# ttwang0303/Adaptive-RGBD-Localization-Mappig

Hardware: AMD Instinct MI355X
Metric: frames/sec (extract+match+RANSAC-PnP) @640x480, 2000 kp (higher is better)
Workload: dtype u8/i32 (extract, match), f32+f64 (ransac, pnp)

## Files before the change

adaptive-rgbd-localization-mappig_amd/csrc/k_extract.hip:

```cpp
#include "odo_device.h"
#include "odo_internal.h"
#ifdef FS_STATS
#include <cstdio>
#endif

#ifndef ODO_EXTRACT_PRIO
#define ODO_EXTRACT_PRIO 0
#endif
#define EXTRACT_PRIO() \
    if (ODO_EXTRACT_PRIO) __builtin_amdgcn_s_setprio(ODO_EXTRACT_PRIO)

namespace odo {

__global__ void __launch_bounds__(256) k_gray(const uint8_t* __restrict__ bgr, uint8_t* __restrict__ pyr,
                                              int w, int h, int pitch, size_t in_stride, size_t pyr_stride) {
    EXTRACT_PRIO();
    const int f = blockIdx.y;
    const int q = blockIdx.x * blockDim.x + threadIdx.x;
    const uint8_t* src = bgr + (size_t)f * in_stride;
    uint8_t* dst = pyr + (size_t)f * pyr_stride;
    const int npix = w * h;
    const int p0 = q * 4;
    if (p0 >= npix) return;
    const int y = p0 / w, x = p0 - y * w;
// ... 35 lines not shown
    const int nrow = min(rb, dh - y0);
    const int t = threadIdx.x;
    uint8_t* base = pyr + (size_t)f * pyr_stride;
    const int sy_lo = yt[y0].sy0, sy_hi = yt[y0 + nrow - 1].sy1;
    const int srows = sy_hi - sy_lo + 1;
    const int nq = (dw + 3) >> 2;
    ResizeX* xs = reinterpret_cast<ResizeX*>(rz_lds);
    uint8_t* rows = rz_lds + (size_t)nq * 4 * sizeof(ResizeX);
    for (int i = t; i < dw; i += 256) xs[i] = xt[i];
    {
        const uint4* src = reinterpret_cast<const uint4*>(base + src_off + (size_t)sy_lo * spitch);
        uint4* dstl = reinterpret_cast<uint4*>(rows);
        const int n16 = srows * (spitch >> 4);
        for (int i = t; i < n16; i += 256) dstl[i] = src[i];
    }
    __syncthreads();
    const float inv_nq = 1.0f / (float)nq;
    const int items = nrow * nq;
    for (int it = t; it < items; it += 256) {
        const int r = (int)(((float)it + 0.5f) * inv_nq);
        const int q = it - r * nq;
        const ResizeY Y = yt[y0 + r];
        const uint8_t* r0 = rows + (uint32_t)__umul24((uint32_t)(Y.sy0 - sy_lo), (uint32_t)spitch);
        const uint8_t* r1 = rows + (uint32_t)__umul24((uint32_t)(Y.sy1 - sy_lo), (uint32_t)spitch);
        const uint32_t b0 = (uint32_t)Y.b0, b1 = (uint32_t)Y.b1;
        uint32_t packed = 0;
#pragma unroll
        for (int j = 0; j < 4; j++) {
            const int dx = 4 * q + j;
            if (dx < dw) {
                const ResizeX X = xs[dx];
                const uint32_t a0 = (uint32_t)X.a0, a1 = (uint32_t)X.a1;
                const uint32_t h0 = __umul24(r0[X.sx0], a0) + __umul24(r0[X.sx1], a1);
                const uint32_t h1 = __umul24(r1[X.sx0], a0) + __umul24(r1[X.sx1], a1);
                const uint32_t v = (__umul24(h0, b0) + __umul24(h1, b1) + (1u << 21)) >> 22;
                packed |= min(v, 255u) << (8 * j);
            }
        }
        *reinterpret_cast<uint32_t*>(base + dst_off + (size_t)(y0 + r) * dpitch + 4 * q) = packed;
    }
}

constexpr int kCircleDx[16] = {0, 1, 2, 3, 3, 3, 2, 1, 0, -1, -2, -3, -3, -3, -2, -1};
constexpr int kCircleDy[16] = {3, 3, 2, 1, 0, -1, -2, -3, -3, -3, -2, -1, 0, 1, 2, 3};
#define FS_TH 256
#define FS_RING 512
#define FS_RSTRIDE (FS_RING + 8)
#define FS_CL 1024

ODO_INLINE void wave_lds_sync() {
    __builtin_amdgcn_fence(__ATOMIC_RELEASE, "wavefront");
    __builtin_amdgcn_wave_barrier();
    __builtin_amdgcn_fence(__ATOMIC_ACQUIRE, "wavefront");
}

#ifdef FS_STATS
__device__ unsigned long long fs_stats[8];
#define FS_STAT(i, v) atomicAdd(&fs_stats[i], (unsigned long long)(v))
#else
#define FS_STAT(i, v) ((void)0)
#endif
ODO_INLINE uint32_t fs_msb_mask(uint32_t b4) {
    return ((b4 & 1u) << 7) | ((b4 & 2u) << 14) | ((b4 & 4u) << 21) | ((b4 & 8u) << 28);
}
ODO_INLINE int wave_incl_scan(int x) {
    x += __builtin_amdgcn_update_dpp(0, x, 0x111, 0xf, 0xf, true);
    x += __builtin_amdgcn_update_dpp(0, x, 0x112, 0xf, 0xf, true);
    x += __builtin_amdgcn_update_dpp(0, x, 0x114, 0xf, 0xf, true);
    x += __builtin_amdgcn_update_dpp(0, x, 0x118, 0xf, 0xf, true);
    x += __builtin_amdgcn_update_dpp(0, x, 0x142, 0xa, 0xf, false);
    x += __builtin_amdgcn_update_dpp(0, x, 0x143, 0xc, 0xf, false);
    return x;
}
struct FastMisc {
    int ncl, ovf, nl;
    int tot[FS_NCM], retry[FS_NCM];
};

__global__ void __launch_bounds__(FS_TH) k_fast_seg(const uint8_t* __restrict__ pyr, size_t pyr_stride,
                                                   const FastSeg* __restrict__ segs, const LevelDesc* __restrict__ lv,
                                                   uint32_t* __restrict__ cand, int* __restrict__ cand_cnt, int ncells,
                                                   int cell_cap, int ini_th, int min_th, FastLds LO) {
    EXTRACT_PRIO();
    extern __shared__ __attribute__((aligned(16))) uint8_t fs_lds[];
    const FastSeg G = segs[blockIdx.x];
    const int f = blockIdx.y;
    const int t = threadIdx.x, lane = t & 63, wave = t >> 6;
    uint8_t* const roi = fs_lds;
    const uint32_t* const roi32 = reinterpret_cast<const uint32_t*>(fs_lds);
    uint8_t* const score = fs_lds + LO.img;
    uint16_t* const ring = reinterpret_cast<uint16_t*>(fs_lds + LO.ring) + wave * FS_RSTRIDE;
    uint16_t* const clist = reinterpret_cast<uint16_t*>(fs_lds + LO.clist);
    uint32_t* const bits = reinterpret_cast<uint32_t*>(fs_lds + LO.bits);
    int* const cnt = reinterpret_cast<int*>(fs_lds + LO.cnt);
    uint2* const qlist = reinterpret_cast<uint2*>(fs_lds + LO.qlist);
    FastMisc& M = *reinterpret_cast<FastMisc*>(fs_lds + LO.misc);
    const LevelDesc L = lv[G.level];
    const int R = G.rows, cols = G.cols, BW = G.bw, wcell = G.wcell, nc = G.ncell;
    constexpr int RS = FS_RS, RS4 = RS >> 2;
    const int sh = G.x0 & 15;
    {
        const uint4* src = reinterpret_cast<const uint4*>(pyr + (size_t)f * pyr_stride + L.off +
                                                          (size_t)G.y0 * L.pitch + (G.x0 & ~15));
        const int nw = (sh + cols + 15) >> 4, p16 = L.pitch >> 4;
        const int rstep = FS_TH / nw, k = t % nw, r0 = t / nw;
        if (r0 < rstep)
            for (int r = r0; r < R; r += rstep)
                reinterpret_cast<uint4*>(roi + r * RS)[k] = src[__umul24((uint32_t)r, (uint32_t)p16) + (uint32_t)k];
        for (int i = t; i < (R * RS) >> 4; i += FS_TH) reinterpret_cast<uint4*>(score)[i] = uint4{0, 0, 0, 0};
        for (int i = t; i < R * BW; i += FS_TH) bits[i] = 0;
        for (int i = t; i < R * FS_NCM; i += FS_TH) cnt[i] = 0;
        if (t == 0) M.ncl = 0, M.ovf = 0;
    }
    const int drows = R - 6;
    const int m0 = (sh + 3) >> 2, m1 = (sh + cols - 4) >> 2;
    {
        const uint32_t mlo = (0xFu << (sh + 3 - 4 * m0)) & 0xFu, mhi = (1u << (sh + cols - 3 - 4 * m1)) - 1u;
        if (t <= m1 - m0) {
            const int m = m0 + t;
            qlist[t] = uint2{fs_msb_mask((t == 0 ? mlo : 0xFu) & (m == m1 ? mhi : 0xFu)), 4u * (uint32_t)m};
        }
    }
    __syncthreads();
    const float inv_w = 1.0f / (float)wcell;
    uint32_t* const out = cand + ((size_t)f * ncells + G.ci0) * cell_cap;
    typedef short s16x2 __attribute__((ext_vector_type(2)));
    for (int pass = 0; pass < 2; pass++) {
        const int th = pass == 0 ? ini_th : min_th;
        const int thc = th < 0 ? 0 : (th > 255 ? 255 : th);
        const int NL = pass == 0 ? m1 - m0 + 1 : M.nl;
        const int items = drows > 0 && cols > 6 && NL > 0 ? drows * NL : 0;
        if (t == 0) FS_STAT(pass, items);
        {
            const s16x2 thv = {(short)thc, (short)thc};
            const float inl = NL > 0 ? 1.0f / (float)NL : 0.0f, inl_h = 0.5f * inl;
            int head = 0, tail = 0;
            auto seg_test = [&](int h, int n) {
                const int i0 = 2 * lane, i1 = i0 + 1;
                bool c0 = false, c1 = false;
                int o0 = 0, o1 = 0;
                if (i0 < n) {
                    o0 = ring[(h + i0) & (FS_RING - 1)];
                    o1 = i1 < n ? ring[(h + i1) & (FS_RING - 1)] : o0;
                    const s16x2 vv = {(short)roi[o0], (short)roi[o1]};
                    int a0 = o0 - 3 * RS - 3, a1 = o1 - 3 * RS - 3;
                    asm("" : "+v"(a0), "+v"(a1));
                    const uint8_t* const q0 = roi + a0;
                    const uint8_t* const q1 = roi + a1;
                    s16x2 d[16];
#pragma unroll
                    for (int k = 0; k < 16; k++) {
                        const int off = (kCircleDy[k] + 3) * RS + kCircleDx[k] + 3;
                        s16x2 c;
                        c.x = (short)q0[off];
                        c.y = (short)q1[off];
                        d[k] = vv - c;
                    }
                    s16x2 mn2[8], mx2[8], mn4[8], mx4[8];
#pragma unroll
                    for (int q = 0; q < 8; q++) {
                        const int j = 2 * q + 1;
                        mn2[q] = __builtin_elementwise_min(d[j], d[(j + 1) & 15]);
                        mx2[q] = __builtin_elementwise_max(d[j], d[(j + 1) & 15]);
                    }
#pragma unroll
                    for (int q = 0; q < 8; q++) {
                        mn4[q] = __builtin_elementwise_min(mn2[q], mn2[(q + 1) & 7]);
                        mx4[q] = __builtin_elementwise_max(mx2[q], mx2[(q + 1) & 7]);
                    }
                    s16x2 dk = s16x2{-32768, -32768}, br = s16x2{32767, 32767};
#pragma unroll
                    for (int q = 0; q < 8; q++) {
                        const int k = 2 * q;
                        const s16x2 m8 = __builtin_elementwise_min(mn4[q], mn4[(q + 2) & 7]);
                        const s16x2 x8 = __builtin_elementwise_max(mx4[q], mx4[(q + 2) & 7]);
                        dk = __builtin_elementwise_max(
                            dk, __builtin_elementwise_min(m8, __builtin_elementwise_max(d[k], d[(k + 9) & 15])));
                        br = __builtin_elementwise_min(
                            br, __builtin_elementwise_max(x8, __builtin_elementwise_min(d[k], d[(k + 9) & 15])));
                    }
                    const s16x2 sc = __builtin_elementwise_max(dk, -br);
                    c0 = sc.x > thc;
                    c1 = i1 < n && sc.y > thc;
                    if (c0) score[o0] = (uint8_t)(sc.x - 1);
                    if (c1) score[o1] = (uint8_t)(sc.y - 1);
                }
                const uint64_t b0 = __ballot(c0), b1 = __ballot(c1);
                const int nco = __popcll(b0) + __popcll(b1);
                if (lane == 0) FS_STAT(3, 1);
                if (nco) {
                    int cb = 0;
                    if (lane == 0) cb = atomicAdd(&M.ncl, nco);
                    cb = __shfl(cb, 0);
                    const int pre = (int)__builtin_amdgcn_mbcnt_hi((uint32_t)(b0 >> 32), __builtin_amdgcn_mbcnt_lo((uint32_t)b0, 0)) +
                                    (int)__builtin_amdgcn_mbcnt_hi((uint32_t)(b1 >> 32), __builtin_amdgcn_mbcnt_lo((uint32_t)b1, 0));
                    const int p0 = cb + pre, p1 = p0 + (c0 ? 1 : 0);
                    if (c0) { if (p0 < FS_CL) clist[p0] = (uint16_t)o0; else M.ovf = 1; }
                    if (c1) { if (p1 < FS_CL) clist[p1] = (uint16_t)o1; else M.ovf = 1; }
                }
            };
            for (int base = wave * 64; base < items; base += FS_TH) {
                uint32_t pass4 = 0;
                int qoff = 0;
                const int it = base + lane;
                if (it < items) {
                    const int ii = (int)__builtin_fmaf((float)it, inl, inl_h);
                    const int kk = it - __mul24(ii, NL);
                    const uint2 e = qlist[kk];
                    int wb = (int)__umul24((uint32_t)ii, (uint32_t)RS) + (int)e.y;
                    asm("" : "+v"(wb));
                    qoff = wb + 3 * RS;
                    const uint32_t* w = reinterpret_cast<const uint32_t*>(roi + wb);
                    const uint32_t Cw = w[3 * RS4], Uw = w[0], Dw = w[6 * RS4];
                    const uint32_t Lw = __builtin_amdgcn_alignbyte(Cw, w[3 * RS4 - 1], 1);
                    const uint32_t Rw = __builtin_amdgcn_alignbyte(w[3 * RS4 + 1], Cw, 3);
                    uint32_t hm[2];
#pragma unroll
                    for (int hh = 0; hh < 2; hh++) {
                        const uint32_t sel = hh ? 0x0c030c02u : 0x0c010c00u;
                        s16x2 v, a0, a4, a8, a12;
                        *reinterpret_cast<uint32_t*>(&v) = __builtin_amdgcn_perm(0u, Cw, sel);
                        *reinterpret_cast<uint32_t*>(&a0) = __builtin_amdgcn_perm(0u, Dw, sel);
                        *reinterpret_cast<uint32_t*>(&a4) = __builtin_amdgcn_perm(0u, Rw, sel);
                        *reinterpret_cast<uint32_t*>(&a8) = __builtin_amdgcn_perm(0u, Uw, sel);
                        *reinterpret_cast<uint32_t*>(&a12) = __builtin_amdgcn_perm(0u, Lw, sel);
                        const s16x2 dk = __builtin_elementwise_max(__builtin_elementwise_min(a0, a8),
                                                                   __builtin_elementwise_min(a4, a12));
                        const s16x2 bk = __builtin_elementwise_min(__builtin_elementwise_max(a0, a8),
                                                                   __builtin_elementwise_max(a4, a12));
                        const s16x2 t1 = dk - (v - thv), t2 = (v + thv) - bk;
                        hm[hh] = *reinterpret_cast<const uint32_t*>(&t1) | *reinterpret_cast<const uint32_t*>(&t2);
                    }
                    pass4 = __builtin_amdgcn_perm(hm[1], hm[0], 0x07050301u) & e.x;
                }
                uint32_t pos = (uint32_t)tail;
#pragma unroll
                for (int k = 0; k < 4; k++) {
                    const bool sv = (pass4 >> (8 * k + 7)) & 1u;
                    const uint64_t bk = __ballot(sv);
                    const uint32_t slot =
                        __builtin_amdgcn_mbcnt_hi((uint32_t)(bk >> 32), __builtin_amdgcn_mbcnt_lo((uint32_t)bk, pos)) &
                        (FS_RING - 1);
                    uint32_t at;
                    asm("v_cndmask_b32_e64 %0, %1, %2, %3" : "=v"(at) : "v"((uint32_t)FS_RING), "v"(slot), "s"(bk));
                    ring[at] = (uint16_t)(qoff + k);
                    pos += (uint32_t)__popcll(bk);
                }
                tail = (int)pos;
                if (tail - head >= 128) {
                    wave_lds_sync();
                    do {
                        seg_test(head, 128);
                        head += 128;
                    } while (tail - head >= 128);
                    wave_lds_sync();
                }
            }
            if (lane == 0) FS_STAT(2, tail);
            if (tail > head) {
                wave_lds_sync();
                seg_test(head, tail - head);
            }
        }
        __syncthreads();
        const bool ovf = M.ovf != 0;
        const int ncl = min(M.ncl, FS_CL);
        if (t == 0) FS_STAT(4, M.ncl), FS_STAT(5, ovf ? 1 : 0);
        auto locate = [&](int o, int& r, int& xs, int& jl, int& xl, int& xh) {
            r = o / RS;
            xs = (o - r * RS) - sh;
            jl = (int)(((float)(xs - 3) + 0.5f) * inv_w);
            xl = 3 + jl * wcell;
            xh = min(xl + wcell, cols - 3);
        };
        auto nms = [&](int o) {
            int so = o - RS - 1;
            asm("" : "+v"(so));
            const uint8_t* const sb = score + so;
            const int sc = sb[RS + 1];
            int r, xs, jl, xl, xh;
            locate(o, r, xs, jl, xl, xh);
            const int nmid = max((int)sb[1], (int)sb[2 * RS + 1]);
            const int nl = max(max((int)sb[0], (int)sb[RS]), (int)sb[2 * RS]);
            const int nr = max(max((int)sb[2], (int)sb[RS + 2]), (int)sb[2 * RS + 2]);
            const int nb = max(nmid, max(xs - 1 >= xl ? nl : 0, xs + 1 < xh ? nr : 0));
            if (sc > nb) {
                atomicOr(&bits[r * BW + (xs >> 5)], 1u << (xs & 31));
                atomicAdd(&cnt[r * FS_NCM + jl], 1);
            }
        };
        auto scan = [&](auto&& fn) {
            for (int it = t; it < items; it += FS_TH) {
                const int ii2 = it / NL, kk2 = it - ii2 * NL;
                const uint2 e = qlist[kk2];
                const uint32_t msk = e.x;
                const int qo = (3 + ii2) * RS + (int)e.y;
                for (int b = 0; b < 4; b++)
                    if (((msk >> (8 * b + 7)) & 1u) && score[qo + b]) fn(qo + b);
            }
        };
        if (!ovf)
            for (int i = t; i < ncl; i += FS_TH) nms(clist[i]);
        else
            scan(nms);
        __syncthreads();
        for (int j = wave; j < nc; j += FS_TH / 64) {
            if (pass == 1 && !M.retry[j]) continue;
            const int r = 3 + lane;
            const int v = lane < drows ? cnt[r * FS_NCM + j] : 0;
            int incl = v;
#pragma unroll
            for (int o = 1; o < 64; o <<= 1) {
                const int y = __shfl_up(incl, o);
                if (lane >= o) incl += y;
            }
            if (lane < drows) cnt[r * FS_NCM + j] = incl - v;
            if (lane == 63) M.tot[j] = incl;
        }
        __syncthreads();
        auto place = [&](int o) {
            int r, xs, jl, xl, xh;
            locate(o, r, xs, jl, xl, xh);
            const uint32_t* row = bits + r * BW;
            if (!((row[xs >> 5] >> (xs & 31)) & 1u)) return;
            int rank = cnt[r * FS_NCM + jl];
            const int wl = xl >> 5, nwd = (xs >> 5) - wl;
            const uint32_t hm = (1u << (xs & 31)) - 1u;
#pragma unroll
            for (int i = 0; i < 4; i++) {
                uint32_t v = row[wl + i];
                if (i == 0) v &= ~0u << (xl & 31);
                v &= i < nwd ? ~0u : (i == nwd ? hm : 0u);
                rank += __builtin_popcount(v);
            }
            if (rank < cell_cap)
                out[(size_t)jl * cell_cap + rank] = ((uint32_t)score[o] << 24) |
                                                    ((uint32_t)(r + G.y0 - 16) << 12) | (uint32_t)(xs + G.x0 - 16);
        };
        if (!ovf)
            for (int i = t; i < ncl; i += FS_TH) place(clist[i]);
        else
            scan(place);
        if (pass == 0) {
            if (t < nc) M.retry[t] = M.tot[t] == 0;
            __syncthreads();
            if (t < nc && M.retry[t]) FS_STAT(6, 1);
            if (t == 0) FS_STAT(7, nc);
            if (t < nc) {
                const int xa = sh + 3 + t * wcell, xe = sh + min(3 + (t + 1) * wcell, cols - 3);
                if (M.retry[t]) {
                    int at = 0;
                    for (int j = 0; j < t; j++)
                        if (M.retry[j]) {
                            const int ja = sh + 3 + j * wcell, je = sh + min(3 + (j + 1) * wcell, cols - 3);
                            at += ((je - 1) >> 2) - (ja >> 2) + 1;
                        }
                    for (int m = xa >> 2; m <= (xe - 1) >> 2; m++) {
                        const int lo = max(xa - 4 * m, 0), hi = min(xe - 4 * m, 4);
                        qlist[at++] = uint2{fs_msb_mask((0xFu << lo) & ((1u << hi) - 1u)), 4u * (uint32_t)m};
                    }
                } else {
                    cand_cnt[(size_t)f * ncells + G.ci0 + t] = min(M.tot[t], cell_cap);
                }
            }
            if (t == 0) {
                int n = 0;
                for (int j = 0; j < nc; j++)
                    if (M.retry[j]) {
                        const int ja = sh + 3 + j * wcell, je = sh + min(3 + (j + 1) * wcell, cols - 3);
                        n += ((je - 1) >> 2) - (ja >> 2) + 1;
                    }
                M.nl = n;
                M.ncl = 0;
                M.ovf = 0;
            }
            __syncthreads();
            if (M.nl == 0) return;
        } else if (t < nc && M.retry[t]) {
            cand_cnt[(size_t)f * ncells + G.ci0 + t] = min(M.tot[t], cell_cap);
        }
    }
}

struct ONode {
    int16_t x0, y0, x1, y1;
    int32_t cnt;
    int32_t seq;
};

#ifndef OT_THREADS
#define OT_THREADS 256
#endif

#ifndef OT_KB
#define OT_KB 8
#endif
#ifndef OT_RANK_MAX
#define OT_RANK_MAX 512
#endif
#ifdef ODO_OCTREE_PROFILE
#define OT_NSTAMP 48
__device__ unsigned long long g_ot_stamp[2][OT_NSTAMP];
#define OT_STAMP(tag)                                                                                   \
    do {                                                                                                \
        if (threadIdx.x == 0 && s_vars[8] >= 0 && s_vars[8] < OT_NSTAMP)                                \
            g_ot_stamp[s_vars[9]][s_vars[8]++] = ((unsigned long long)(tag) << 56) | (wall_clock64() & 0xFFFFFFFFFFFFFFull); \
    } while (0)
#else
#define OT_STAMP(tag) ((void)0)
#endif
#ifndef OT_HIST_WAVE0
#define OT_HIST_WAVE0 1
#endif
enum { OT_LDK = 1, OT_LDN = 2 };
template <bool RES, int LD, typename F>
ODO_INLINE void ot_pass(int n, int t, uint32_t (&rk)[OT_KB], int (&rn)[OT_KB], const uint32_t* keys, int32_t* knode,
                        F&& f) {
    if constexpr (RES) {
#pragma unroll
        for (int u = 0; u < OT_KB; u++)
            if (t + u * OT_THREADS < n) f(t + u * OT_THREADS, rk[u], rn[u]);
    } else {
        for (int k0 = t; k0 < n; k0 += OT_THREADS * OT_KB) {
#pragma unroll
            for (int u = 0; u < OT_KB; u++) {
                const int k = k0 + u * OT_THREADS;
                rn[u] = -1;
                if (k < n) {
                    if (LD & OT_LDK) rk[u] = keys[k];
                    if (LD & OT_LDN) rn[u] = knode[k];
                }
            }
#pragma unroll
            for (int u = 0; u < OT_KB; u++) {
                const int k = k0 + u * OT_THREADS;
                if (k < n) {
                    int node = rn[u];
                    f(k, rk[u], node);
                    if (node != rn[u]) knode[k] = node;
                }
            }
        }
    }
}

ODO_INLINE int block_exclusive_scan(int v, int* tmp, int* total);

ODO_INLINE int ot_gather(const uint32_t* __restrict__ cand, const int* __restrict__ cand_cnt, size_t cell0, int nc,
                         int cell_cap, uint32_t* dst, int cap, int* scan) {
    const int t = threadIdx.x;
    int n = 0;
    for (int cb = 0; cb < nc; cb += OT_THREADS) {
        const int c = cb + t;
        const int cnt = c < nc ? cand_cnt[cell0 + c] : 0;
        int tot;
        const int ex = block_exclusive_scan(cnt, scan, &tot);
        if (c < nc) {
// ... 1441 lines not shown
```

adaptive-rgbd-localization-mappig_amd/csrc/k_finalize.hip:

```cpp
#include "odo_device.h"
#include "odo_internal.h"
#ifndef ODO_EXTRACT_PRIO
#define ODO_EXTRACT_PRIO 0
#endif
#include "../../include/odo_orb_pattern.h"

namespace odo {

typedef float f32x2 __attribute__((ext_vector_type(2)));

__constant__ float4 c_patf[256];
__constant__ uint32_t c_pat8[256];
__constant__ int c_umax16[16];

#define RND_MAGIC 12582912.0f
#define RND_BITS 0x4B400000u

#define FIN_KPW 4

#define FL_IC_W 9
#define FL_IC_N (31 * FL_IC_W)
#define FL_BR_W 10
#define FL_BR_N (37 * FL_BR_W)
#define FL_KP_RAW FL_BR_N
#define FL_KP_DW (((FL_KP_RAW + 15) / 32) * 32 + 16)
template <int NW>
__global__ void __launch_bounds__(64 * NW) k_finalize_lds(const uint8_t* __restrict__ pyr, const uint8_t* __restrict__ blur,
                                                      size_t pyr_stride, const LevelDesc* __restrict__ lv, int nlevels,
                                                      const uint32_t* __restrict__ okp, const int* __restrict__ ocnt,
                                                      int okp_stride, orb_kp* __restrict__ kps, uint8_t* __restrict__ desc,
                                                      int* __restrict__ nkp, int kp_cap) {
    if (ODO_EXTRACT_PRIO) __builtin_amdgcn_s_setprio(ODO_EXTRACT_PRIO);
    __shared__ uint64_t s_bal[NW][16];
    __shared__ __attribute__((aligned(16))) uint32_t s_disc[16][12];
    __shared__ __attribute__((aligned(16))) uint32_t s_patch[NW * FIN_KPW][FL_KP_DW];
    for (int d = threadIdx.x; d < 128; d += 64 * NW) {
        const int av = d >> 3, i = d & 7;
        const int um = c_umax16[av];
        uint32_t m = 0;
#pragma unroll
        for (int bb = 0; bb < 4; bb++) {
            const int u = 4 * i + bb - 15;
            if (u >= -um && u <= um) m |= 0xffu << (8 * bb);
        }
        s_disc[av][i] = m;
    }
    int bx = blockIdx.x, f = blockIdx.y;
    {
        const int total = gridDim.x * gridDim.y;
        if ((total & 7) == 0) {
            const int h = blockIdx.x + blockIdx.y * gridDim.x;
            const int lid = (h & 7) * (total >> 3) + (h >> 3);
            bx = lid % gridDim.x;
            f = lid / gridDim.x;
        }
    }
    const int wave = threadIdx.x >> 6, lane = threadIdx.x & 63;
    const int g = lane >> 4, sub = lane & 15;
    const int kslot = wave * FIN_KPW + g;
    const int idx = bx * (NW * FIN_KPW) + kslot;
    int lvl = -1, k = 0, acc = 0;
    for (int i = 0; i < nlevels; i++) {
        const int c = ocnt[f * nlevels + i];
        if (lvl < 0 && idx < acc + c) {
            lvl = i;
            k = idx - acc;
        }
        acc += c;
    }
    const int total = acc < kp_cap ? acc : kp_cap;
    if (bx == 0 && threadIdx.x == 0) nkp[f] = total;
    if (bx * (NW * FIN_KPW) >= total) return;
    const bool valid = lvl >= 0 && idx < kp_cap;
    const LevelDesc L = lv[valid ? lvl : 0];
    const uint32_t key = valid ? okp[((size_t)f * nlevels + lvl) * okp_stride + k] : (16u | (16u << 12));
    const int kx = (int)(key & 0xfff) + 16, ky = (int)((key >> 12) & 0xfff) + 16;
    const float resp = (float)(key >> 24);
    constexpr int IC_STEPS = 7, BR_STEPS = 13;
    uint2 vbr[BR_STEPS];
    uint32_t* P = s_patch[kslot];
    const int sh = (kx - 15) & 3, sh2 = (kx - 18) & 3;
    const bool glane = sub < 15;
    const int ir = sub / 3, ic = sub - 3 * ir;
    const int br = sub / 5, bc = sub - 5 * br;
    {
        const uint8_t* fpyr = pyr + (size_t)f * pyr_stride;
        const uint8_t* fblur = blur + (size_t)f * pyr_stride;
        const uint32_t pitch = (uint32_t)L.pitch;
        uint3 v[IC_STEPS];
        {
            const uint32_t o0 = (uint32_t)L.off + (uint32_t)(ky - 15) * pitch + (uint32_t)(kx - 15 - sh);
            uint32_t o = o0 + (uint32_t)ir * pitch + 12u * (uint32_t)ic;
#pragma unroll
            for (int j = 0; j < IC_STEPS; j++) {
                const bool ok = j + 1 < IC_STEPS || ir == 0;
                v[j] = *reinterpret_cast<const uint3*>(fpyr + (ok ? o : o0));
                o += 5u * pitch;
            }
        }
        {
            const uint32_t o0 = (uint32_t)L.off + (uint32_t)(ky - 18) * pitch + (uint32_t)(kx - 18 - sh2);
            uint32_t o = o0 + (uint32_t)br * pitch + 8u * (uint32_t)bc;
#pragma unroll
            for (int j = 0; j < BR_STEPS; j++) {
                const bool ok = j + 1 < BR_STEPS || br == 0;
                vbr[j] = *reinterpret_cast<const uint2*>(fblur + (ok ? o : o0));
                o += 3u * pitch;
            }
        }
        {
            uint32_t* d = P + ir * FL_IC_W + 3 * ic;
#pragma unroll
            for (int j = 0; j < IC_STEPS; j++) {
                if (glane && (j + 1 < IC_STEPS || ir == 0)) {
                    d[0] = v[j].x;
                    d[1] = v[j].y;
                    d[2] = v[j].z;
                }
                d += 5 * FL_IC_W;
            }
        }
    }
    __syncthreads();
    int m10, m01;
    {
        const bool has1 = sub < 15;
        const int v0 = sub - 15, v1 = has1 ? sub + 1 : 0;
        const uint32_t* r0 = P + (v0 + 15) * FL_IC_W;
        const uint32_t* r1 = P + (v1 + 15) * FL_IC_W;
        uint32_t w0[9], w1[9];
#pragma unroll
        for (int i = 0; i < 9; i++) {
            w0[i] = r0[i];
            w1[i] = r1[i];
        }
        const uint4* M0 = reinterpret_cast<const uint4*>(s_disc[-v0]);
        const uint4* M1 = reinterpret_cast<const uint4*>(s_disc[v1]);
        const uint4 a0 = M0[0], a1 = M0[1], b0 = M1[0], b1 = M1[1];
        const uint32_t z = has1 ? 0xffffffffu : 0u;
        const uint32_t mk0[8] = {a0.x, a0.y, a0.z, a0.w, a1.x, a1.y, a1.z, a1.w};
        const uint32_t mk1[8] = {b0.x & z, b0.y & z, b0.z & z, b0.w & z, b1.x & z, b1.y & z, b1.z & z, b1.w & z};
        uint32_t s0 = 0, s1 = 0, t = 0;
#pragma unroll
        for (int i = 0; i < 8; i++) {
            const uint32_t U = (uint32_t)(4 * i + 1) | ((uint32_t)(4 * i + 2) << 8) | ((uint32_t)(4 * i + 3) << 16) |
                               ((uint32_t)(4 * i + 4) << 24);
            const uint32_t d0 = __builtin_amdgcn_alignbyte(w0[i + 1], w0[i], sh) & mk0[i];
            const uint32_t d1 = __builtin_amdgcn_alignbyte(w1[i + 1], w1[i], sh) & mk1[i];
            s0 = __builtin_amdgcn_udot4(d0, 0x01010101u, s0, false);
            s1 = __builtin_amdgcn_udot4(d1, 0x01010101u, s1, false);
            t = __builtin_amdgcn_udot4(d0, U, t, false);
            t = __builtin_amdgcn_udot4(d1, U, t, false);
        }
        m10 = (int)t - 16 * (int)(s0 + s1);
        m01 = v0 * (int)s0 + v1 * (int)s1;
    }
#pragma unroll
    for (int off = 8; off > 0; off >>= 1) {
        m10 += __shfl_xor(m10, off);
        m01 += __shfl_xor(m01, off);
    }
    const float angle = fast_atan2((float)m01, (float)m10);
    const float factorPI = (float)(3.14159265358979323846 / 180.f);
    const float ang = angle * factorPI;
    double sd, cd;
    sincos((double)ang, &sd, &cd);
    const float a = (float)cd, b = (float)sd;
    const f32x2 BA = {b, a}, AB = {a, b}, MAG = {RND_MAGIC, RND_MAGIC};
    __syncthreads();
    {
        uint32_t* d = P + br * FL_BR_W + 2 * bc;
#pragma unroll
        for (int j = 0; j < BR_STEPS; j++) {
            if (glane && (j + 1 < BR_STEPS || br == 0)) *reinterpret_cast<uint2*>(d) = vbr[j];
            d += 3 * FL_BR_W;
        }
    }
    __syncthreads();
    const uint8_t* PB = reinterpret_cast<const uint8_t*>(P);
    const uint32_t cofs = (uint32_t)(18 * 4 * FL_BR_W + 18 + sh2) - 0x400000u * (uint32_t)(4 * FL_BR_W) - RND_BITS;
    int tv0[16], tv1[16];
    uint32_t pat8[16];
#pragma unroll
    for (int u = 0; u < 4; u++) {
        const uint4 q = reinterpret_cast<const uint4*>(c_pat8)[sub * 4 + u];
        pat8[4 * u] = q.x, pat8[4 * u + 1] = q.y, pat8[4 * u + 2] = q.z, pat8[4 * u + 3] = q.w;
    }
#pragma unroll
    for (int w = 0; w < 16; w++) {
        const uint32_t pw = pat8[w];
        const float4 Pt = {(float)(int8_t)(pw & 0xff), (float)(int8_t)((pw >> 8) & 0xff),
                           (float)(int8_t)((pw >> 16) & 0xff), (float)(int8_t)(pw >> 24)};
        f32x2 q0 = (f32x2){Pt.x, Pt.x} * BA + (f32x2){Pt.y, -Pt.y} * AB;
        f32x2 q1 = (f32x2){Pt.z, Pt.z} * BA + (f32x2){Pt.w, -Pt.w} * AB;
        q0 = q0 + MAG;
        q1 = q1 + MAG;
        const uint32_t o0 = __umul24(__float_as_uint(q0.x), (uint32_t)(4 * FL_BR_W)) + __float_as_uint(q0.y) + cofs;
        const uint32_t o1 = __umul24(__float_as_uint(q1.x), (uint32_t)(4 * FL_BR_W)) + __float_as_uint(q1.y) + cofs;
        tv0[w] = PB[o0];
        tv1[w] = PB[o1];
    }
#pragma unroll
    for (int w = 0; w < 16; w++) {
        const uint64_t bal = __ballot(tv0[w] < tv1[w]);
        if (lane == 0) s_bal[wave][w] = bal;
    }
    __syncthreads();
    const int o = idx;
    if (valid && sub < 8) {
        const uint32_t lo = (uint32_t)(s_bal[wave][2 * sub] >> (16 * g)) & 0xffffu;
        const uint32_t hi = (uint32_t)(s_bal[wave][2 * sub + 1] >> (16 * g)) & 0xffffu;
        reinterpret_cast<uint32_t*>(desc + ((size_t)f * kp_cap + o) * 32)[sub] = lo | (hi << 16);
    }
    if (valid && sub == 0) {
        orb_kp* kp = kps + (size_t)f * kp_cap + o;
        float px = (float)kx, py = (float)ky;
        if (lvl != 0) {
            px *= L.scale;
            py *= L.scale;
        }
        kp->x = px;
        kp->y = py;
        kp->size = (float)(int)(31 * L.scale);
        kp->angle = angle;
        kp->response = resp;
        kp->octave = lvl;
        kp->class_id = -1;
    }
}

__global__ void __launch_bounds__(256) k_kp_geometry(const orb_kp* __restrict__ kps, const int* __restrict__ nkp,
                                                     const uint16_t* __restrict__ depth, size_t depth_stride, int img_w,
                                                     FrameCalib cal, float* __restrict__ kun, float* __restrict__ xyz,
                                                     float* __restrict__ ur, int kp_cap) {
    const int f = blockIdx.y, i = blockIdx.x * blockDim.x + threadIdx.x;
    if (i >= nkp[f]) return;
    const size_t o = (size_t)f * kp_cap + i;
    const float2 p = *reinterpret_cast<const float2*>(&kps[o].x);
    kp_geometry(p.x, p.y, cal, depth + (size_t)f * depth_stride, img_w, kun + o * 2, xyz + o * 3, ur + o);
}

void upload_finalize_constants() {
    float4 pat[256];
    for (int t = 0; t < 256; t++)
        pat[t] = make_float4((float)ODO_ORB_PATTERN[4 * t], (float)ODO_ORB_PATTERN[4 * t + 1],
                             (float)ODO_ORB_PATTERN[4 * t + 2], (float)ODO_ORB_PATTERN[4 * t + 3]);
    hipMemcpyToSymbol(HIP_SYMBOL(c_patf), pat, sizeof(pat));
    uint32_t pat8[256];
    for (int sl = 0; sl < 16; sl++)
        for (int w = 0; w < 16; w++) {
            const int t = w * 16 + sl;
            uint32_t v = 0;
            for (int i = 0; i < 4; i++) v |= (uint32_t)(uint8_t)(int8_t)ODO_ORB_PATTERN[4 * t + i] << (8 * i);
            pat8[sl * 16 + w] = v;
        }
    hipMemcpyToSymbol(HIP_SYMBOL(c_pat8), pat8, sizeof(pat8));
    const int umax[16] = {15, 15, 15, 15, 14, 14, 14, 13, 13, 12, 11, 10, 9, 8, 6, 3};
    hipMemcpyToSymbol(HIP_SYMBOL(c_umax16), umax, sizeof(umax));
}

void launch_kp_geometry(hipStream_t st, const orb_kp* kps, const int* nkp, const uint16_t* depth, size_t depth_stride,
                        int img_w, FrameCalib cal, float* kun, float* xyz, float* ur, int kp_cap, int nframes) {
    dim3 g((kp_cap + 255) / 256, nframes);
    hipLaunchKernelGGL(k_kp_geometry, g, dim3(256), 0, st, kps, nkp, depth, depth_stride, img_w, cal, kun, xyz, ur,
                       kp_cap);
}

void launch_finalize(hipStream_t st, const uint8_t* pyr, const uint8_t* blur, size_t pyr_stride, const LevelDesc* lv,
                     int nlevels, const uint32_t* okp, const int* ocnt, int okp_stride, const uint16_t* depth,
                     size_t depth_stride, int img_w, FrameCalib cal, orb_kp* kps, uint8_t* desc, float* kun, float* xyz,
                     float* ur, int* nkp, int kp_cap, int nframes, bool geometry) {
    hipLaunchKernelGGL(k_finalize_lds<2>, dim3((kp_cap + 7) / 8, nframes), dim3(128), 0, st, pyr, blur, pyr_stride, lv,
                       nlevels, okp, ocnt, okp_stride, kps, desc, nkp, kp_cap);
    if (geometry) launch_kp_geometry(st, kps, nkp, depth, depth_stride, img_w, cal, kun, xyz, ur, kp_cap, nframes);
}

}
```

adaptive-rgbd-localization-mappig_amd/csrc/odo_geometry.cpp:

```cpp
#include "odo_ctx.h"

inline int cvRoundH(float v) { return (int)lrintf(v); }
inline int cvFloorH(float v) {
    int i = (int)v;
    return i - (i > v);
}
inline int satShort(float v) {
    int r = cvRoundH(v);
    return std::min(std::max(r, -32768), 32767);
}

static int build_adaptive_orb_geometry(odo_ctx* c) {
    const odo_adaptive_params& P = c->cfg.adaptive;
    float scale[OA_NLEV];
    int quota[OA_NLEV];
    {
        const double sf = (double)1.2f;
        const float factor = (float)(1.0 / sf);
        float nd = 10000 * (1 - factor) / (1 - (float)pow((double)factor, (double)OA_NLEV));
        int sum = 0;
        for (int l = 0; l < OA_NLEV; l++) {
            scale[l] = (float)pow(sf, (double)l);
            c->osc.s[l] = scale[l];
            if (l < OA_NLEV - 1) {
// ... 160 lines not shown
    for (int l = 0; l < p.nlevels - 1; l++) {
        quota[l] = cvRoundH(nDesired);
        sum += quota[l];
        nDesired *= factor;
    }
    quota[p.nlevels - 1] = std::max(p.nfeatures - sum, 0);

    c->lv_h.resize(p.nlevels);
    int off = 0, maxq = 0, max_nini = 1;
    size_t key_off = 0;
    c->cells_h.clear();
    c->fsegs_h.clear();
    int max_tiles = 0;
    for (int l = 0; l < p.nlevels; l++) {
        LevelDesc& L = c->lv_h[l];
        L.w = cvRoundH((float)W * inv[l]);
        L.h = cvRoundH((float)H * inv[l]);
        L.pitch = (L.w + 15) & ~15;
        L.off = off;
        L.scale = scale[l];
        L.quota = quota[l];
        off += L.pitch * L.h;
        maxq = std::max(maxq, quota[l]);
        if (L.w < 40 || L.h < 40) return fail(ODO_ERR_ARG, "pyramid level too small (< 40 px)");
        const float Wc = 30;
        const int minBorderX = 16, minBorderY = 16;
        const int maxBorderX = L.w - 16, maxBorderY = L.h - 16;
        const float width = (float)(maxBorderX - minBorderX), height = (float)(maxBorderY - minBorderY);
        const int nCols = (int)(width / Wc), nRows = (int)(height / Wc);
        const int wCell = (int)ceil(width / nCols), hCell = (int)ceil(height / nRows);
        L.cell_begin = (int)c->cells_h.size();
        for (int i = 0; i < nRows; i++) {
            const float iniY = (float)(minBorderY + i * hCell);
            float maxY = iniY + hCell + 6;
            if (iniY >= maxBorderY - 3) continue;
            if (maxY > maxBorderY) maxY = (float)maxBorderY;
            for (int j = 0; j < nCols; j++) {
                const float iniX = (float)(minBorderX + j * wCell);
                float maxX = iniX + wCell + 6;
                if (iniX >= maxBorderX - 6) continue;
                if (maxX > maxBorderX) maxX = (float)maxBorderX;
                CellDesc C;
                C.level = (int16_t)l;
                C.y0 = (int16_t)(int)iniY;
                C.x0 = (int16_t)(int)iniX;
                C.rows = (int16_t)((int)maxY - (int)iniY);
                C.cols = (int16_t)((int)maxX - (int)iniX);
                C.offx = (int16_t)(j * wCell);
                C.offy = (int16_t)(i * hCell);
                C.pad = 0;
                if (C.rows > FAST_ROI_MAX || C.cols > FAST_ROI_MAX) return fail(ODO_ERR_ARG, "FAST cell exceeds ROI max");
                c->cells_h.push_back(C);
                c->fast_roi = std::max(c->fast_roi, (int)std::max(C.rows, C.cols));
                c->cell_cap = std::max(c->cell_cap, ((C.rows - 6 + 1) / 2) * ((C.cols - 6 + 1) / 2) + 1);
            }
        }
        L.cell_end = (int)c->cells_h.size();
        {
            const int nct = L.cell_end - L.cell_begin;
            int ncj = 0;
            for (int j = 0; j < nCols; j++)
                if ((float)(minBorderX + j * wCell) < (float)(maxBorderX - 6)) ncj++;
            if (ncj > 0 && nct % ncj == 0) {
                const int kmax = std::min(FS_SEGC, (FS_RS - 15 - 6) / wCell);
                if (kmax < 1) return fail(ODO_ERR_ARG, "FAST cell wider than a segment row");
                const int nrow = nct / ncj, nseg = (ncj + kmax - 1) / kmax;
                for (int ir = 0; ir < nrow; ir++)
                    for (int sg = 0; sg < nseg; sg++) {
                        const int ja = ncj * sg / nseg, jb = ncj * (sg + 1) / nseg;
                        const CellDesc& A = c->cells_h[L.cell_begin + ir * ncj + ja];
                        const CellDesc& B = c->cells_h[L.cell_begin + ir * ncj + jb - 1];
                        FastSeg G{};
                        G.level = l;
                        G.ci0 = L.cell_begin + ir * ncj + ja;
                        G.y0 = A.y0;
                        G.rows = A.rows;
                        G.x0 = A.x0;
                        G.cols = (int16_t)(B.x0 + B.cols - A.x0);
                        G.ncell = (int16_t)(jb - ja);
                        G.wcell = (int16_t)wCell;
                        G.bw = (int16_t)((G.cols + 31) >> 5);
                        if ((A.x0 & 15) + G.cols > FS_RS || G.ncell > FS_NCM || G.rows > 70 || (int)G.rows * FS_RS > 65536)
                            return fail(ODO_ERR_ARG, "FAST segment too large");
                        c->fsegs_h.push_back(G);
                    }
            } else if (nct > 0) {
                return fail(ODO_ERR_STATE, "FAST cells not a full grid");
            }
        }
        L.key_off = (int)key_off;
        const int nIni = (int)roundf((float)(maxBorderX - minBorderX) / (float)(maxBorderY - minBorderY));
        max_nini = std::max(max_nini, nIni);
        const int tiles = ((L.w + 63) / 64) * ((L.h + 15) / 16);
        max_tiles = std::max(max_tiles, tiles);
    }
    c->ncells = (int)c->cells_h.size();
    c->cell_cap = (c->cell_cap + 3) & ~3;
    for (int l = 0; l < p.nlevels; l++) {
        LevelDesc& L = c->lv_h[l];
        L.key_off = 0;
    }
    size_t koff = 0;
    for (int l = 0; l < p.nlevels; l++) {
        c->lv_h[l].key_off = (int)koff;
        koff += (size_t)(c->lv_h[l].cell_end - c->lv_h[l].cell_begin) * c->cell_cap;
    }
    c->keys_per_frame = koff;
    c->pyr_size = (size_t)off + 64;
    c->max_blur_tiles = max_tiles;
    c->okp_stride = maxq + 8;
    int nc = 64;
    while (nc < std::max(maxq + 8, 4 * max_nini + 8)) nc <<= 1;
    c->node_cap = nc;
    if (octree_lds_bytes(nc) > 160 * 1024) return fail(ODO_ERR_ARG, "octree node capacity exceeds LDS");
    c->kp_cap = ((p.nfeatures + 4 * p.nlevels + 8) + 63) & ~63;
    if (c->kp_cap > 8192) return fail(ODO_ERR_ARG, "nfeatures too large (kp cap 8192)");
    if (c->adaptive) {
        int e;
        if ((e = build_adaptive_geometry(c))) return e;
        if (c->kp_cap > 8192) return fail(ODO_ERR_ARG, "ADAPTIVE max_total_keypoints too large (kp cap 8192)");
    }
    c->match_cap = c->kp_cap;
    c->mask_words = (c->match_cap + 31) / 32;
    std::vector<ResizeX> rx;
    std::vector<ResizeY> ry;
    c->rx_off.assign(p.nlevels, 0);
    c->ry_off.assign(p.nlevels, 0);
    c->rz_rows.assign(p.nlevels, 0);
    for (int l = 1; l < p.nlevels; l++) {
        const LevelDesc& S = c->lv_h[l - 1];
        const LevelDesc& D = c->lv_h[l];
        const double inv_sx = (double)D.w / S.w, inv_sy = (double)D.h / S.h;
        const double scale_x = 1. / inv_sx, scale_y = 1. / inv_sy;
        c->rx_off[l] = (int)rx.size();
        std::vector<int> xofs(D.w);
        std::vector<int> a0(D.w), a1(D.w);
        int xmax = D.w;
        for (int dx = 0; dx < D.w; dx++) {
            float fx = (float)((dx + 0.5) * scale_x - 0.5);
            int sx = cvFloorH(fx);
            fx -= sx;
            if (sx < 0) {
                fx = 0;
                sx = 0;
            }
            if (sx + 1 >= S.w) {
                xmax = std::min(xmax, dx);
                if (sx >= S.w - 1) {
                    fx = 0;
                    sx = S.w - 1;
                }
            }
            xofs[dx] = sx;
            a0[dx] = satShort((1.f - fx) * 2048);
            a1[dx] = satShort(fx * 2048);
        }
        for (int dx = 0; dx < D.w; dx++) {
            ResizeX X;
            X.sx0 = xofs[dx];
            if (dx < xmax) {
                X.sx1 = xofs[dx] + 1;
                X.a0 = a0[dx];
                X.a1 = a1[dx];
            } else {
                X.sx1 = xofs[dx];
                X.a0 = 2048;
// ... 46 lines not shown
```

adaptive-rgbd-localization-mappig_amd/csrc/odo_internal.h:

```cpp
#pragma once

#include <hip/hip_runtime.h>
#include <stddef.h>
#include <stdint.h>
#include <stdlib.h>

#include "../../include/odo_types.h"

namespace odo {

static inline const char* odo_knob(const char* name) {
#ifdef ODO_TUNING
    return getenv(name);
#else
    (void)name;
    return nullptr;
#endif
}

#define FAST_ROI_MAX 72

struct LevelDesc {
    int off;
    int w, h;
    int pitch;
    float scale;
    int quota;
    int cell_begin;
    int cell_end;
    int key_off;
};

struct CellDesc {
    int16_t level;
    int16_t rows, cols;
    int16_t x0, y0;
    int16_t offx, offy;
    int16_t pad;
};

#ifndef FS_SEGC
#define FS_SEGC 8
#endif
#define FS_NCM FS_SEGC
#ifndef FS_RS
#define FS_RS 272
#endif
struct FastSeg {
    int level, ci0;
    int16_t y0, x0, rows, cols, ncell, wcell;
    int16_t bw, pad;
};
struct FastLds {
    int img;
    int ring, clist, bits, cnt, qlist, misc, total;
};

struct ResizeX {
    int sx0, sx1;
    int a0, a1;
};
struct ResizeY {
    int sy0, sy1;
    int b0, b1;
};

struct FrameCalib {
    float fx, fy, cx, cy;
    float k1, k2, p1, p2, k3;
    float depth_factor, mbf;
    float invfx, invfy;
};

__device__ inline void kp_geometry(float uu, float vv, const FrameCalib& cal, const uint16_t* depth, int img_w,
                                   float* ku, float* p3, float* urp) {
    float ux = uu, uy = vv;
    if (cal.k1 != 0.0f) {
        const double fx = cal.fx, fy = cal.fy, cx = cal.cx, cy = cal.cy;
        const double ifx = 1. / fx, ify = 1. / fy;
        const double k0 = cal.k1, k1 = cal.k2, k2 = cal.p1, k3 = cal.p2, k4 = cal.k3;
        double x = uu, y = vv;
        x = (x - cx) * ifx;
        y = (y - cy) * ify;
        const double x0 = x, y0 = y;
        for (int j = 0; j < 5; j++) {
            double r2 = x * x + y * y;
            double icdist = 1 / (1 + ((k4 * r2 + k1) * r2 + k0) * r2);
            double deltaX = 2 * k2 * x * y + k3 * (r2 + 2 * x * x);
            double deltaY = k2 * (r2 + 2 * y * y) + 2 * k3 * x * y;
            x = (x0 - deltaX) * icdist;
            y = (y0 - deltaY) * icdist;
        }
        ux = (float)(fx * x + cx);
        uy = (float)(fy * y + cy);
    }
    ku[0] = ux;
    ku[1] = uy;
    float urv = -1.f, X = 0.f, Y = 0.f, Z = 0.f;
    const uint16_t d16 = depth[(size_t)((int)vv) * img_w + (int)uu];
    const float z = (float)d16 * cal.depth_factor + 0.0f;
    if (z > 0) {
        urv = ux - cal.mbf / z;
        X = (ux - cal.cx) * z * cal.invfx;
        Y = (uy - cal.cy) * z * cal.invfy;
        Z = z;
    }
    p3[0] = X;
    p3[1] = Y;
    p3[2] = Z;
    *urp = urv;
}

#define AD_BH 16
#define AD_MAXW 1024
#define AD_SEL_LDS 4096
using AdParams = odo_adaptive_params;

struct AdCell {
    int rs, re, cs, ce;
    int r0, r1, c0, c1;
    int band0, band1;
    int cand_cap;
    int pad;
};
struct AdBand {
    int cell, y0, y1, cand_off;
};

#define OA_NLEV 8
#define OA_EDGE 15
#define OA_PATCH 31
#ifndef OA_BH
#define OA_BH 64
#endif
struct OaImg {
// ... 299 lines not shown
```

Measured before the change: 164,000.

## Precompute FAST segment staging params and trim integer divides in extract kernels

Moves per-block FAST segment values (row step, division magic, inverse cell width) into the host-built segment descriptor, which the kernel now loads as two 16-byte vectors. The kernel replaces integer divides and modulo with multiply-shift forms, merges the LDS zeroing loops, and rebuilds the pass-0 retry list with a single-wave scan instead of serial loops. In the finalize kernel, the disc mask table becomes a compile-time constant, the level lookup is unrolled, the grid remap uses a precomputed reciprocal, and ballots are batched. These changes add assumptions tied to FS_TH==256 and RS==272, plus a VGPR clobber that may change register allocation.

After: 166,800, median of 6. 1.7% higher.

```diff
diff --git a/adaptive-rgbd-localization-mappig_amd/csrc/k_extract.hip b/adaptive-rgbd-localization-mappig_amd/csrc/k_extract.hip
--- a/adaptive-rgbd-localization-mappig_amd/csrc/k_extract.hip
+++ b/adaptive-rgbd-localization-mappig_amd/csrc/k_extract.hip
@@ -141,8 +141,16 @@
                                                    uint32_t* __restrict__ cand, int* __restrict__ cand_cnt, int ncells,
                                                    int cell_cap, int ini_th, int min_th, FastLds LO) {
     EXTRACT_PRIO();
+#ifndef FS_FREE_VGPRS
+    asm volatile("" ::: "v79");
+#endif
     extern __shared__ __attribute__((aligned(16))) uint8_t fs_lds[];
-    const FastSeg G = segs[blockIdx.x];
+    FastSeg G;
+    {
+        const uint4* const gp = reinterpret_cast<const uint4*>(segs + blockIdx.x);
+        const uint4 g2[2] = {gp[0], gp[1]};
+        __builtin_memcpy(&G, g2, sizeof(G));
+    }
     const int f = blockIdx.y;
     const int t = threadIdx.x, lane = t & 63, wave = t >> 6;
     uint8_t* const roi = fs_lds;
@@ -159,16 +167,22 @@
     constexpr int RS = FS_RS, RS4 = RS >> 2;
     const int sh = G.x0 & 15;
     {
-        const uint4* src = reinterpret_cast<const uint4*>(pyr + (size_t)f * pyr_stride + L.off +
-                                                          (size_t)G.y0 * L.pitch + (G.x0 & ~15));
-        const int nw = (sh + cols + 15) >> 4, p16 = L.pitch >> 4;
-        const int rstep = FS_TH / nw, k = t % nw, r0 = t / nw;
-        if (r0 < rstep)
-            for (int r = r0; r < R; r += rstep)
-                reinterpret_cast<uint4*>(roi + r * RS)[k] = src[__umul24((uint32_t)r, (uint32_t)p16) + (uint32_t)k];
+        static_assert(FS_TH == 256, "fast_seg_staging sizes the grid for 256 threads");
+        const uint8_t* const src = pyr + (size_t)f * pyr_stride + L.off + (size_t)G.y0 * L.pitch + (G.x0 & ~15);
+        const uint32_t nw = (uint32_t)G.nw, rstep = (uint32_t)G.rstep, pitch = (uint32_t)L.pitch;
+        const uint32_t r0 = __umul24((uint32_t)t, (uint32_t)G.rmag) >> 12, k = (uint32_t)t - __umul24(r0, nw);
+        if (r0 < rstep) {
+            uint32_t so = __umul24(r0, pitch) + 16u * k, lo = __umul24(r0, (uint32_t)RS) + 16u * k;
+            const uint32_t sstep = __umul24(rstep, pitch), lstep = __umul24(rstep, (uint32_t)RS);
+            for (uint32_t r = r0; r < (uint32_t)R; r += rstep, so += sstep, lo += lstep)
+                *reinterpret_cast<uint4*>(roi + lo) = *reinterpret_cast<const uint4*>(src + so);
+        }
         for (int i = t; i < (R * RS) >> 4; i += FS_TH) reinterpret_cast<uint4*>(score)[i] = uint4{0, 0, 0, 0};
-        for (int i = t; i < R * BW; i += FS_TH) bits[i] = 0;
-        for (int i = t; i < R * FS_NCM; i += FS_TH) cnt[i] = 0;
+        {
+            uint4* const z = reinterpret_cast<uint4*>(bits);
+            const int nz = (LO.cnt - LO.bits + R * FS_NCM * 4 + 15) >> 4;
+            for (int i = t; i < nz; i += FS_TH) z[i] = uint4{0, 0, 0, 0};
+        }
         if (t == 0) M.ncl = 0, M.ovf = 0;
     }
     const int drows = R - 6;
@@ -181,7 +195,7 @@
         }
     }
     __syncthreads();
-    const float inv_w = 1.0f / (float)wcell;
+    const float inv_w = G.inv_w;
     uint32_t* const out = cand + ((size_t)f * ncells + G.ci0) * cell_cap;
     typedef short s16x2 __attribute__((ext_vector_type(2)));
     for (int pass = 0; pass < 2; pass++) {
@@ -192,7 +206,7 @@
         if (t == 0) FS_STAT(pass, items);
         {
             const s16x2 thv = {(short)thc, (short)thc};
-            const float inl = NL > 0 ? 1.0f / (float)NL : 0.0f, inl_h = 0.5f * inl;
+            const float inl = NL > 0 ? __builtin_amdgcn_rcpf((float)NL) : 0.0f, inl_h = 0.5f * inl;
             int head = 0, tail = 0;
             auto seg_test = [&](int h, int n) {
                 const int i0 = 2 * lane, i1 = i0 + 1;
@@ -326,8 +340,11 @@
         const int ncl = min(M.ncl, FS_CL);
         if (t == 0) FS_STAT(4, M.ncl), FS_STAT(5, ovf ? 1 : 0);
         auto locate = [&](int o, int& r, int& xs, int& jl, int& xl, int& xh) {
-            r = o / RS;
-            xs = (o - r * RS) - sh;
+            if constexpr (RS == 272)
+                r = (int)(__umul24((uint32_t)o, 61681u) >> 24);
+            else
+                r = o / RS;
+            xs = (o - __mul24(r, RS)) - sh;
             jl = (int)(((float)(xs - 3) + 0.5f) * inv_w);
             xl = 3 + jl * wcell;
             xh = min(xl + wcell, cols - 3);
@@ -367,12 +384,7 @@
             if (pass == 1 && !M.retry[j]) continue;
             const int r = 3 + lane;
             const int v = lane < drows ? cnt[r * FS_NCM + j] : 0;
-            int incl = v;
-#pragma unroll
-            for (int o = 1; o < 64; o <<= 1) {
-                const int y = __shfl_up(incl, o);
-                if (lane >= o) incl += y;
-            }
+            const int incl = wave_incl_scan(v);
             if (lane < drows) cnt[r * FS_NCM + j] = incl - v;
             if (lane == 63) M.tot[j] = incl;
         }
@@ -401,37 +413,31 @@
         else
             scan(place);
         if (pass == 0) {
-            if (t < nc) M.retry[t] = M.tot[t] == 0;
-            __syncthreads();
-            if (t < nc && M.retry[t]) FS_STAT(6, 1);
-            if (t == 0) FS_STAT(7, nc);
-            if (t < nc) {
-                const int xa = sh + 3 + t * wcell, xe = sh + min(3 + (t + 1) * wcell, cols - 3);
-                if (M.retry[t]) {
-                    int at = 0;
-                    for (int j = 0; j < t; j++)
-                        if (M.retry[j]) {
-                            const int ja = sh + 3 + j * wcell, je = sh + min(3 + (j + 1) * wcell, cols - 3);
-                            at += ((je - 1) >> 2) - (ja >> 2) + 1;
+            if (ovf) __syncthreads();
+            if (wave == 0) {
+                int lane = t;
+                asm volatile("" : "+v"(lane));
+                const bool cell = lane < nc;
+                const int tot = cell ? M.tot[lane] : 1;
+                const bool rt = tot == 0;
+                const int xa = sh + 3 + lane * wcell, xe = sh + min(3 + (lane + 1) * wcell, cols - 3);
+                const int nq = rt ? ((xe - 1) >> 2) - (xa >> 2) + 1 : 0;
+                const int incl = wave_incl_scan(nq);
+                if (lane == 0) FS_STAT(7, nc);
+                if (cell) {
+                    M.retry[lane] = rt;
+                    if (rt) {
+                        FS_STAT(6, 1);
+                        int at = incl - nq;
+                        for (int m = xa >> 2; m <= (xe - 1) >> 2; m++) {
+                            const int lo = max(xa - 4 * m, 0), hi = min(xe - 4 * m, 4);
+                            qlist[at++] = uint2{fs_msb_mask((0xFu << lo) & ((1u << hi) - 1u)), 4u * (uint32_t)m};
                         }
-                    for (int m = xa >> 2; m <= (xe - 1) >> 2; m++) {
-                        const int lo = max(xa - 4 * m, 0), hi = min(xe - 4 * m, 4);
-                        qlist[at++] = uint2{fs_msb_mask((0xFu << lo) & ((1u << hi) - 1u)), 4u * (uint32_t)m};
+                    } else {
+                        cand_cnt[(size_t)f * ncells + G.ci0 + lane] = min(tot, cell_cap);
                     }
-                } else {
-                    cand_cnt[(size_t)f * ncells + G.ci0 + t] = min(M.tot[t], cell_cap);
-                }
-            }
-            if (t == 0) {
-                int n = 0;
-                for (int j = 0; j < nc; j++)
-                    if (M.retry[j]) {
-                        const int ja = sh + 3 + j * wcell, je = sh + min(3 + (j + 1) * wcell, cols - 3);
-                        n += ((je - 1) >> 2) - (ja >> 2) + 1;
-                    }
-                M.nl = n;
-                M.ncl = 0;
-                M.ovf = 0;
+                }
+                if (lane == 63) M.nl = incl, M.ncl = 0, M.ovf = 0;
             }
             __syncthreads();
             if (M.nl == 0) return;
diff --git a/adaptive-rgbd-localization-mappig_amd/csrc/k_finalize.hip b/adaptive-rgbd-localization-mappig_amd/csrc/k_finalize.hip
--- a/adaptive-rgbd-localization-mappig_amd/csrc/k_finalize.hip
+++ b/adaptive-rgbd-localization-mappig_amd/csrc/k_finalize.hip
@@ -9,9 +9,25 @@
 
 typedef float f32x2 __attribute__((ext_vector_type(2)));
 
-__constant__ float4 c_patf[256];
 __constant__ uint32_t c_pat8[256];
-__constant__ int c_umax16[16];
+struct DiscTab {
+    uint32_t m[16 * 8];
+};
+constexpr DiscTab make_disc_tab() {
+    constexpr int umax[16] = {15, 15, 15, 15, 14, 14, 14, 13, 13, 12, 11, 10, 9, 8, 6, 3};
+    DiscTab T{};
+    for (int av = 0; av < 16; av++)
+        for (int i = 0; i < 8; i++) {
+            uint32_t m = 0;
+            for (int bb = 0; bb < 4; bb++) {
+                const int u = 4 * i + bb - 15;
+                if (u >= -umax[av] && u <= umax[av]) m |= 0xffu << (8 * bb);
+            }
+            T.m[av * 8 + i] = m;
+        }
+    return T;
+}
+__constant__ DiscTab c_disc = make_disc_tab();
 
 #define RND_MAGIC 12582912.0f
 #define RND_BITS 0x4B400000u
@@ -29,50 +45,52 @@
                                                       size_t pyr_stride, const LevelDesc* __restrict__ lv, int nlevels,
                                                       const uint32_t* __restrict__ okp, const int* __restrict__ ocnt,
                                                       int okp_stride, orb_kp* __restrict__ kps, uint8_t* __restrict__ desc,
-                                                      int* __restrict__ nkp, int kp_cap) {
+                                                      int* __restrict__ nkp, int kp_cap, uint32_t gx_rcp) {
     if (ODO_EXTRACT_PRIO) __builtin_amdgcn_s_setprio(ODO_EXTRACT_PRIO);
     __shared__ uint64_t s_bal[NW][16];
     __shared__ __attribute__((aligned(16))) uint32_t s_disc[16][12];
     __shared__ __attribute__((aligned(16))) uint32_t s_patch[NW * FIN_KPW][FL_KP_DW];
-    for (int d = threadIdx.x; d < 128; d += 64 * NW) {
-        const int av = d >> 3, i = d & 7;
-        const int um = c_umax16[av];
-        uint32_t m = 0;
-#pragma unroll
-        for (int bb = 0; bb < 4; bb++) {
-            const int u = 4 * i + bb - 15;
-            if (u >= -um && u <= um) m |= 0xffu << (8 * bb);
-        }
-        s_disc[av][i] = m;
-    }
+    for (int d = threadIdx.x; d < 128; d += 64 * NW) s_disc[d >> 3][d & 7] = c_disc.m[d];
     int bx = blockIdx.x, f = blockIdx.y;
     {
-        const int total = gridDim.x * gridDim.y;
-        if ((total & 7) == 0) {
-            const int h = blockIdx.x + blockIdx.y * gridDim.x;
-            const int lid = (h & 7) * (total >> 3) + (h >> 3);
-            bx = lid % gridDim.x;
-            f = lid / gridDim.x;
+        const uint32_t gx = gridDim.x, total = gx * gridDim.y;
+        if ((total & 7) == 0 && gx_rcp != 0) {
+            const uint32_t h = blockIdx.x + blockIdx.y * gx;
+            const uint32_t lid = (h & 7) * (total >> 3) + (h >> 3);
+            f = (int)__umulhi(lid, gx_rcp);
+            bx = (int)(lid - (uint32_t)f * gx);
         }
     }
     const int wave = threadIdx.x >> 6, lane = threadIdx.x & 63;
     const int g = lane >> 4, sub = lane & 15;
     const int kslot = wave * FIN_KPW + g;
     const int idx = bx * (NW * FIN_KPW) + kslot;
-    int lvl = -1, k = 0, acc = 0;
-    for (int i = 0; i < nlevels; i++) {
-        const int c = ocnt[f * nlevels + i];
-        if (lvl < 0 && idx < acc + c) {
-            lvl = i;
-            k = idx - acc;
-        }
-        acc += c;
-    }
+    int lvl = 0, acc = 0;
+    uint32_t ku = (uint32_t)idx;
+    {
+        const int* const oc = ocnt + f * nlevels;
+        int c8[8];
+#pragma unroll
+        for (int i = 0; i < 8; i++) c8[i] = oc[i < nlevels ? i : nlevels - 1];
+#pragma unroll
+        for (int i = 0; i < 8; i++) {
+            acc += i < nlevels ? c8[i] : 0;
+            lvl += idx >= acc ? 1 : 0;
+            ku = min(ku, (uint32_t)idx - (uint32_t)acc);
+        }
+        for (int i = 8; i < nlevels; i++) {
+            acc += oc[i];
+            lvl += idx >= acc ? 1 : 0;
+            ku = min(ku, (uint32_t)idx - (uint32_t)acc);
+        }
+    }
+    const int k = (int)ku;
     const int total = acc < kp_cap ? acc : kp_cap;
     if (bx == 0 && threadIdx.x == 0) nkp[f] = total;
     if (bx * (NW * FIN_KPW) >= total) return;
-    const bool valid = lvl >= 0 && idx < kp_cap;
-    const LevelDesc L = lv[valid ? lvl : 0];
+    const bool valid = idx < acc && idx < kp_cap;
+    if (!valid) lvl = 0;
+    const LevelDesc L = lv[lvl];
     const uint32_t key = valid ? okp[((size_t)f * nlevels + lvl) * okp_stride + k] : (16u | (16u << 12));
     const int kx = (int)(key & 0xfff) + 16, ky = (int)((key >> 12) & 0xfff) + 16;
     const float resp = (float)(key >> 24);
@@ -200,10 +218,15 @@
         tv0[w] = PB[o0];
         tv1[w] = PB[o1];
     }
-#pragma unroll
-    for (int w = 0; w < 16; w++) {
-        const uint64_t bal = __ballot(tv0[w] < tv1[w]);
-        if (lane == 0) s_bal[wave][w] = bal;
+    uint64_t bal[16];
+#pragma unroll
+    for (int w = 0; w < 16; w++) bal[w] = __ballot(tv0[w] < tv1[w]);
+    if (lane == 0) {
+#pragma unroll
+        for (int w = 0; w < 16; w++) {
+            s_bal[wave][w] = bal[w];
+            asm volatile("" ::: "memory");
+        }
     }
     __syncthreads();
     const int o = idx;
@@ -241,11 +264,6 @@
 }
 
 void upload_finalize_constants() {
-    float4 pat[256];
-    for (int t = 0; t < 256; t++)
-        pat[t] = make_float4((float)ODO_ORB_PATTERN[4 * t], (float)ODO_ORB_PATTERN[4 * t + 1],
-                             (float)ODO_ORB_PATTERN[4 * t + 2], (float)ODO_ORB_PATTERN[4 * t + 3]);
-    hipMemcpyToSymbol(HIP_SYMBOL(c_patf), pat, sizeof(pat));
     uint32_t pat8[256];
     for (int sl = 0; sl < 16; sl++)
         for (int w = 0; w < 16; w++) {
@@ -255,8 +273,6 @@
             pat8[sl * 16 + w] = v;
         }
     hipMemcpyToSymbol(HIP_SYMBOL(c_pat8), pat8, sizeof(pat8));
-    const int umax[16] = {15, 15, 15, 15, 14, 14, 14, 13, 13, 12, 11, 10, 9, 8, 6, 3};
-    hipMemcpyToSymbol(HIP_SYMBOL(c_umax16), umax, sizeof(umax));
 }
 
 void launch_kp_geometry(hipStream_t st, const orb_kp* kps, const int* nkp, const uint16_t* depth, size_t depth_stride,
@@ -270,8 +286,11 @@
                      int nlevels, const uint32_t* okp, const int* ocnt, int okp_stride, const uint16_t* depth,
                      size_t depth_stride, int img_w, FrameCalib cal, orb_kp* kps, uint8_t* desc, float* kun, float* xyz,
                      float* ur, int* nkp, int kp_cap, int nframes, bool geometry) {
-    hipLaunchKernelGGL(k_finalize_lds<2>, dim3((kp_cap + 7) / 8, nframes), dim3(128), 0, st, pyr, blur, pyr_stride, lv,
-                       nlevels, okp, ocnt, okp_stride, kps, desc, nkp, kp_cap);
+    const uint32_t gx = (uint32_t)(kp_cap + 7) / 8;
+    const uint64_t ntot = (uint64_t)gx * (uint64_t)nframes;
+    const uint32_t gx_rcp = gx > 1 && ntot * gx < (1ull << 32) ? (uint32_t)(((1ull << 32) + gx - 1) / gx) : 0u;
+    hipLaunchKernelGGL(k_finalize_lds<2>, dim3(gx, nframes), dim3(128), 0, st, pyr, blur, pyr_stride, lv, nlevels, okp,
+                       ocnt, okp_stride, kps, desc, nkp, kp_cap, gx_rcp);
     if (geometry) launch_kp_geometry(st, kps, nkp, depth, depth_stride, img_w, cal, kun, xyz, ur, kp_cap, nframes);
 }
 
diff --git a/adaptive-rgbd-localization-mappig_amd/csrc/odo_geometry.cpp b/adaptive-rgbd-localization-mappig_amd/csrc/odo_geometry.cpp
--- a/adaptive-rgbd-localization-mappig_amd/csrc/odo_geometry.cpp
+++ b/adaptive-rgbd-localization-mappig_amd/csrc/odo_geometry.cpp
@@ -266,6 +266,7 @@
                         G.bw = (int16_t)((G.cols + 31) >> 5);
                         if ((A.x0 & 15) + G.cols > FS_RS || G.ncell > FS_NCM || G.rows > 70 || (int)G.rows * FS_RS > 65536)
                             return fail(ODO_ERR_ARG, "FAST segment too large");
+                        fast_seg_staging(G);
                         c->fsegs_h.push_back(G);
                     }
             } else if (nct > 0) {
diff --git a/adaptive-rgbd-localization-mappig_amd/csrc/odo_internal.h b/adaptive-rgbd-localization-mappig_amd/csrc/odo_internal.h
--- a/adaptive-rgbd-localization-mappig_amd/csrc/odo_internal.h
+++ b/adaptive-rgbd-localization-mappig_amd/csrc/odo_internal.h
@@ -49,8 +49,18 @@
 struct FastSeg {
     int level, ci0;
     int16_t y0, x0, rows, cols, ncell, wcell;
-    int16_t bw, pad;
-};
+    int16_t bw;
+    int16_t nw, rstep, rmag;
+    float inv_w;
+};
+static_assert(sizeof(FastSeg) == 32, "FastSeg is read as two uint4");
+inline void fast_seg_staging(FastSeg& G) {
+    const int nw = ((G.x0 & 15) + G.cols + 15) >> 4;
+    G.nw = (int16_t)nw;
+    G.rstep = (int16_t)(256 / nw);
+    G.rmag = (int16_t)((4096 + nw - 1) / nw);
+    G.inv_w = 1.0f / (float)G.wcell;
+}
 struct FastLds {
     int img;
     int ring, clist, bits, cnt, qlist, misc, total;
```
